# microsoft/fadtk

Hardware: AMD Instinct MI355X
Metric: FAD scores/sec + cov-GEMM TFLOP/s (% MFMA peak), N=100k D=512 (higher is better)
Workload: dtype f16 in, f16 MFMA with f32 accumulate over <= 8192-row runs, f64 across runs (moments); split-f16 MFMA iterations (f32 accumulate) + exact int8-MFMA products (int32 accumulate) + f64 correction (Frechet)

## Files before the change

### fadtk_amd/csrc/moments_kernels.h

```cpp
#pragma once
#include "fad_common.h"
#include <type_traits>

namespace fad {

typedef float f32x16 __attribute__((ext_vector_type(16)));
typedef double f64x4 __attribute__((ext_vector_type(4)));
typedef _Float16 f16x8 __attribute__((ext_vector_type(8)));
typedef __bf16 bf16x8 __attribute__((ext_vector_type(8)));
typedef short s16x4 __attribute__((ext_vector_type(4)));

constexpr int kXcd = 8;
constexpr int kMaxSets = 16;
constexpr int kMaxSets256 = 32;

__device__ __forceinline__ int xcd_contiguous(int b, int nwg) {
    const int xcd = b % kXcd, idx = b / kXcd;
    const int q = nwg / kXcd, r = nwg % kXcd;
    return (xcd < r ? xcd * (q + 1) : r * (q + 1) + (xcd - r) * q) + idx;
}

__device__ __forceinline__ void tile_coords(int tile, int nt, int& ta, int& tb) {
    int a = 0, t = tile;
    while (t >= nt - a) { t -= nt - a; ++a; }
    ta = a; tb = a + t;
}

struct SegRun;
struct TileSet {
    const void* E;
    int64_t n, ld;
    int64_t rows_per_split;
    int S;
    int item0;
    void* partials;
    double* colpart;
    int* flag;
    uint16_t* cvec;
    const SegRun* runs;
    const int* split_first_run;
    float* seg_runsum;
};
struct SegRun { int64_t r0; int32_t rows; int32_t seg; };
struct TileLaunch {
    TileSet set[kMaxSets];
    int nsets, d, nt, T, total;
};

__device__ __forceinline__ const TileSet& locate(const TileLaunch& L, int w, int& split, int& tile, int64_t& k_begin,
                                                 int64_t& k_end, int& run_lo, int& run_hi) {
    int si = 0;
#pragma unroll
    for (int i = 1; i < kMaxSets; ++i)
        if (i < L.nsets && w >= L.set[i].item0) si = i;
    const TileSet& s = L.set[si];
    const int local = w - s.item0;
    split = local / L.T; tile = local - split * L.T;
    k_begin = (int64_t)split * s.rows_per_split;
    k_end = (k_begin + s.rows_per_split < s.n) ? k_begin + s.rows_per_split : s.n;
    run_lo = 0; run_hi = 0;
    if (s.runs) { run_lo = s.split_first_run[split]; run_hi = s.split_first_run[split + 1]; }
    return s;
}

template <int KIND> __device__ __forceinline__ float h16_to_f32(uint32_t bits16) {
    if constexpr (KIND == FAD_F16) {
        _Float16 h; unsigned short s = (unsigned short)bits16; __builtin_memcpy(&h, &s, 2); return (float)h;
    } else {
        return __uint_as_float(bits16 << 16);
    }
}

template <int KIND> __device__ __forceinline__ float sum8(const uint4& v) {
    float s = 0.f;
    const uint32_t w[4] = {v.x, v.y, v.z, v.w};
#pragma unroll
    for (int q = 0; q < 4; ++q) {
        if constexpr (KIND == FAD_F16) {
            typedef _Float16 h2 __attribute__((ext_vector_type(2)));
            h2 a; __builtin_memcpy(&a, &w[q], 4);
            const h2 one = {(_Float16)1.0f, (_Float16)1.0f};
            s = __builtin_amdgcn_fdot2(a, one, s, false);
        } else {
            typedef __bf16 b2 __attribute__((ext_vector_type(2)));
            b2 a, one; __builtin_memcpy(&a, &w[q], 4);
            const uint32_t ob = 0x3f803f80u; __builtin_memcpy(&one, &ob, 4);
            s = __builtin_amdgcn_fdot2_f32_bf16(a, one, s, false);
        }
    }
    return s;
}

template <int KIND> __device__ __forceinline__ f32x16 mfma_h16(const uint4& a, const uint4& b, const f32x16& c) {
    if constexpr (KIND == FAD_F16) {
        f16x8 va, vb; __builtin_memcpy(&va, &a, 16); __builtin_memcpy(&vb, &b, 16);
        return __builtin_amdgcn_mfma_f32_32x32x16_f16(va, vb, c, 0, 0, 0);
    } else {
        bf16x8 va, vb; __builtin_memcpy(&va, &a, 16); __builtin_memcpy(&vb, &b, 16);
        return __builtin_amdgcn_mfma_f32_32x32x16_bf16(va, vb, c, 0, 0, 0);
    }
}

constexpr int H_BT = 128;
constexpr int H_TS = H_BT * H_BT + 64;
constexpr int H_KB = 32;
constexpr int H_NST = 4;

__device__ __attribute__((aligned(16))) uint4 g_zero16 = {0u, 0u, 0u, 0u};

typedef const void __attribute__((address_space(1)))* gptr_t;
typedef void __attribute__((address_space(3)))* lptr_t;

template <int N> __device__ __forceinline__ void wait_vmcnt() {
    asm volatile("s_waitcnt vmcnt(%0)" ::"n"(N) : "memory");
}

template <int N> __device__ __forceinline__ void wait_vmcnt_upto(int outstanding_steps) {
    switch (outstanding_steps) {
        case 0: wait_vmcnt<0>(); break;
        case 1: wait_vmcnt<N>(); break;
        case 2: wait_vmcnt<2 * N>(); break;
        case 3: wait_vmcnt<3 * N>(); break;
        case 4: wait_vmcnt<4 * N>(); break;
        case 5: wait_vmcnt<5 * N>(); break;
        case 6: wait_vmcnt<6 * N>(); break;
        default: wait_vmcnt<7 * N>(); break;
    }
}

template <int KIND, int NST, bool DIAG, bool FAST, bool SHIFT = false, bool WALK = false>
__device__ __forceinline__ void tile_h16_tr_body(
    const uint16_t* __restrict__ E, int64_t k_begin0, int64_t k_end0, int64_t ld, int d, int nt, int T,
    int split, int tile, int ca, int cb, float* __restrict__ partials, double* __restrict__ colpart,
    uint4* smem, int* __restrict__ shift_flag, const SegRun* __restrict__ runs, int run_lo, int run_hi,
    uint16_t* __restrict__ cvec = nullptr, float* __restrict__ seg_runsum = nullptr) {
    static_assert(!WALK || (DIAG && !SHIFT), "the per-file walk rides on the diagonal tiles of the first pass");
    static_assert(!SHIFT || KIND == FAD_F16, "the shifted pass is written for float16 rows");
    constexpr int LPS = DIAG ? 2 : 4;
    constexpr int STAGE = FAST ? 2 * H_KB * 16 : H_KB * 16;
    static_assert(FAST || DIAG, "single-tile launches only have the diagonal tile");
    const int tid = threadIdx.x, lane = tid & 63;
    const int wave = __builtin_amdgcn_readfirstlane(tid >> 6);
    const int wr = wave >> 1, wc = wave & 1;
    const int li = lane & 31, kg = lane >> 5;
    int64_t k_begin = k_begin0, k_end = k_end0;
    int nkb = 0;

    const int sr = tid >> 4, sc = (tid & 15) ^ (((tid >> 4) & 3) << 2);
    const bool col_ok_a = (ca + sc * 8) < d;
    const bool col_ok_b = (cb + sc * 8) < d;
    const uint16_t* ga = E + ca + sc * 8;
    const uint16_t* gb = E + cb + sc * 8;
    const uint16_t* zsrc = reinterpret_cast<const uint16_t*>(&g_zero16);
    const int t16 = lane & 15, grp = lane >> 4;
    const int tr_row = 8 * (grp >> 1) + (t16 >> 2);
    const int tr_col = 16 * (grp & 1) + 4 * (t16 & 3);

    auto issue_part = [&](int kb, int g) {
        uint4* st = smem + (kb % NST) * STAGE;
        const int h = DIAG ? g : (g >> 1);
        const int64_t r = k_begin + (int64_t)kb * H_KB + sr + 16 * h;
        const bool ok = r < k_end;
        const bool side_b = !DIAG && (g & 1);
        const uint16_t* src = side_b ? ((ok && col_ok_b) ? gb + r * ld : zsrc) : ((ok && col_ok_a) ? ga + r * ld : zsrc);
        uint4* dstp = st + 256 * h + 64 * wave + (side_b ? H_KB * 16 : 0);
        if (FAST) {
            const uint32_t m0v = __builtin_amdgcn_readfirstlane((uint32_t)(size_t)(lptr_t)dstp);
            asm volatile("s_mov_b32 m0, %1\n\ts_nop 0\n\tglobal_load_lds_dwordx4 %0, off" ::"v"(src), "s"(m0v) : "memory", "m0");
        } else {
            __builtin_amdgcn_global_load_lds((gptr_t)src, (lptr_t)dstp, 16, 0, 0);
        }
    };
    auto issue = [&](int kb) {
#pragma unroll
        for (int g = 0; g < LPS; ++g) issue_part(kb, g);
    };
    const bool cols_full = (ca + H_BT <= d) && (cb + H_BT <= d) && ld < ((int64_t)1 << 26);
    const uint32_t voff = (uint32_t)(((int64_t)sr * ld + sc * 8) * 2);
    const uint32_t smem_lds = (uint32_t)(size_t)(lptr_t)smem;
    auto issue_fast = [&](int kb) {
#pragma unroll
        for (int g = 0; g < LPS; ++g) {
            const int h = DIAG ? g : (g >> 1);
            const bool side_b = !DIAG && (g & 1);
            const uint64_t sb = (uint64_t)(E + (k_begin + (int64_t)kb * H_KB + 16 * h) * ld + (side_b ? cb : ca));
            const uint32_t lo = __builtin_amdgcn_readfirstlane((uint32_t)sb);
            const uint32_t hi = __builtin_amdgcn_readfirstlane((uint32_t)(sb >> 32));
            const uint64_t ub = ((uint64_t)hi << 32) | lo;
            const uint32_t dst = smem_lds + (uint32_t)(((kb % NST) * STAGE + 256 * h + 64 * wave + (side_b ? H_KB * 16 : 0)) * 16);
            const uint32_t m0v = __builtin_amdgcn_readfirstlane(dst);
            asm volatile("s_mov_b32 m0, %2\n\ts_nop 0\n\tglobal_load_lds_dwordx4 %0, %1" ::"v"(voff), "s"(ub), "s"(m0v) : "memory", "m0");
        }
    };
    int nfast = 0;

    f32x16 acc[2][2];
#pragma unroll
    for (int x = 0; x < 2; ++x)
#pragma unroll
        for (int y = 0; y < 2; ++y)
#pragma unroll
            for (int q = 0; q < 16; ++q) acc[x][y][q] = 0.f;
    double csum[2] = {0.0, 0.0};
    double ctot[2] = {0.0, 0.0};
    const bool do_colsum = DIAG && (wr == wc);

    auto frag = [&](const char* slab, int ks, int col0) -> uint4 {
        const int r0 = ks * 16 + tr_row, r1 = r0 + 4, col = col0 + tr_col;
        const int o0 = r0 * 256 + (((col >> 3) ^ ((r0 & 3) << 2)) << 4) + ((col >> 2) & 1) * 8;
        const int o1 = r1 * 256 + (((col >> 3) ^ ((r1 & 3) << 2)) << 4) + ((col >> 2) & 1) * 8;
        const s16x4 lo = __builtin_amdgcn_ds_read_tr16_b64_v4i16((__attribute__((address_space(3))) s16x4*)(slab + o0));
        const s16x4 hi = __builtin_amdgcn_ds_read_tr16_b64_v4i16((__attribute__((address_space(3))) s16x4*)(slab + o1));
        uint4 f;
        __builtin_memcpy(&f.x, &lo, 8);
        __builtin_memcpy(&f.z, &hi, 8);
        return f;
    };
    auto split2 = [&](uint4 f, uint32_t c2, int64_t rows_left, uint4& xs, uint4& es) {
        typedef _Float16 h2 __attribute__((ext_vector_type(2)));
        uint32_t w[4] = {f.x, f.y, f.z, f.w}, x[4], e[4];
        h2 c; __builtin_memcpy(&c, &c2, 4);
        const h2 b = -c;
#pragma unroll
        for (int q = 0; q < 4; ++q) {
            h2 a; __builtin_memcpy(&a, &w[q], 4);
            const h2 sm = a + b;
            const h2 bb = sm - a;
            const h2 er = (a - (sm - bb)) + (b - bb);
            __builtin_memcpy(&x[q], &sm, 4);
            __builtin_memcpy(&e[q], &er, 4);
            if (rows_left < 8) {
                const uint32_t m = ((2 * q < rows_left) ? 0xffffu : 0u) | ((2 * q + 1 < rows_left) ? 0xffff0000u : 0u);
                x[q] &= m; e[q] &= m;
            }
        }
        xs = make_uint4(x[0], x[1], x[2], x[3]);
        es = make_uint4(e[0], e[1], e[2], e[3]);
    };
    uint32_t cs[4] = {0u, 0u, 0u, 0u};
    if constexpr (SHIFT) {
        const uint16_t* cv = cvec + (int64_t)split * (nt * H_BT);
        const bool four = DIAG && (wr != wc);
        const int col[4] = {four ? ca + li : ca + 64 * wr + li, four ? ca + 32 + li : ca + 64 * wr + 32 + li,
                            four ? ca + 64 + li : cb + 64 * wc + li, four ? ca + 96 + li : cb + 64 * wc + 32 + li};
#pragma unroll
        for (int q = 0; q < 4; ++q) { const uint32_t h = cv[col[q]]; cs[q] = h | (h << 16); }
    }
    auto rows_left_at = [&](int kb, int ks) -> int64_t { return k_end - (k_begin + (int64_t)kb * H_KB + ks * 16 + 8 * kg); };
    auto load_frags = [&](int kb, int ks, uint4 (&F)[4], uint4 (&R)[4], bool full) {
        const char* sA = reinterpret_cast<const char*>(smem + (kb % NST) * STAGE);
        const char* sB = DIAG ? sA : sA + H_KB * 256;
        F[0] = frag(sA, ks, 64 * wr); F[1] = frag(sA, ks, 64 * wr + 32);
// ... 1062 lines not shown
```

### fadtk_amd/csrc/moments_tile256.h

```cpp
#pragma once
#include "moments_kernels.h"
#include "tile256_roles.h"

namespace fad {

constexpr int T2_KB = 32;
#ifndef T2_NST_VALUE
#define T2_NST_VALUE 4
#endif
constexpr int T2_NST = T2_NST_VALUE;
constexpr int T2_ROW = 1024;
constexpr int T2_STAGE = T2_KB * T2_ROW;
constexpr size_t kT256Lds = (size_t)T2_NST * T2_STAGE;

struct T256Set {
    const void* E; int64_t n, ld, rows_per_split;
    int S, item0;
    float* partials;
    double* colpart;
    int* flag;
    uint16_t* cvec;
    const int32_t* idx; int64_t n_src;
};
struct T256Launch {
    T256Set set[kMaxSets256];
    int nsets, d, nsb, NT, total;
    uint8_t type[t256::MAX_TYPES], sa[t256::MAX_TYPES], sb[t256::MAX_TYPES];
};

__device__ __forceinline__ void t2_phase_barrier() {
    __builtin_amdgcn_sched_barrier(0);
    __builtin_amdgcn_s_barrier();
    __builtin_amdgcn_sched_barrier(0);
}

__device__ __forceinline__ uint4 t2_frag(uint32_t lds_byte) {
    typedef __attribute__((address_space(3))) s16x4* lp_t;
    const s16x4 lo = __builtin_amdgcn_ds_read_tr16_b64_v4i16((lp_t)(size_t)lds_byte);
    const s16x4 hi = __builtin_amdgcn_ds_read_tr16_b64_v4i16((lp_t)(size_t)(lds_byte + 4 * T2_ROW));
    uint4 f;
    __builtin_memcpy(&f.x, &lo, 8);
    __builtin_memcpy(&f.z, &hi, 8);
    return f;
}

__device__ __forceinline__ void t2_split2(const uint4& f, uint32_t c2, int64_t rows_left, uint4& xs, uint4& es) {
    typedef _Float16 h2 __attribute__((ext_vector_type(2)));
    uint32_t w[4] = {f.x, f.y, f.z, f.w}, x[4], e[4];
    h2 c; __builtin_memcpy(&c, &c2, 4);
    const h2 b = -c;
#pragma unroll
    for (int q = 0; q < 4; ++q) {
        h2 a; __builtin_memcpy(&a, &w[q], 4);
        const h2 sm = a + b;
        const h2 bb = sm - a;
        const h2 er = (a - (sm - bb)) + (b - bb);
        __builtin_memcpy(&x[q], &sm, 4);
        __builtin_memcpy(&e[q], &er, 4);
        if (rows_left < 8) {
            const uint32_t m = ((2 * q < rows_left) ? 0xffffu : 0u) | ((2 * q + 1 < rows_left) ? 0xffff0000u : 0u);
            x[q] &= m; e[q] &= m;
        }
    }
    xs = make_uint4(x[0], x[1], x[2], x[3]);
    es = make_uint4(e[0], e[1], e[2], e[3]);
}

template <int KIND, int ROLE, bool SHIFT, bool IDX>
__device__ __forceinline__ void tile256_wave(
    const T256Launch& L, const T256Set& s, int split, int ti, int type, int sa, int sb, const t256::WaveJob job, char* smem) {
    using RD = t256::RoleDef<ROLE>;
    constexpr int NF = RD::NF, NB = RD::NB;
    static_assert(!SHIFT || KIND == FAD_F16, "the shifted pass is written for float16 rows");
    constexpr int NSTG = T2_NST;
    constexpr int LPS = 4;
    const int tid = threadIdx.x, lane = tid & 63;
    const int wave = __builtin_amdgcn_readfirstlane(tid >> 6);
    const int quartet = wave >> 2;
    const int li = lane & 31, kg = lane >> 5;
    const uint16_t* __restrict__ E = static_cast<const uint16_t*>(s.E);
    const int64_t ld = s.ld;
    const int d = L.d;
    const bool two_rows = type == t256::TYPE_Z;
    const int64_t k_begin = (int64_t)split * s.rows_per_split;
    const int64_t k_end = (k_begin + s.rows_per_split < s.n) ? k_begin + s.rows_per_split : s.n;
    const int rows_per_stage = two_rows ? 2 * T2_KB : T2_KB;
    const int nkb = (int)((k_end - k_begin + rows_per_stage - 1) / rows_per_stage);
    const int colA = t256::SB * sa, colB = t256::SB * (two_rows ? sa : sb);
    const int my_rowoff = two_rows ? T2_KB * quartet : 0;

    typedef int srd_t __attribute__((ext_vector_type(4)));
    srd_t srd;
    {
        const uint64_t b = (uint64_t)(IDX ? E : E + k_begin * ld);
        const uint64_t nbytes = (uint64_t)(((IDX ? s.n_src : k_end - k_begin) - 1) * ld + d) * 2;
        srd[0] = __builtin_amdgcn_readfirstlane((int)(uint32_t)b);
        srd[1] = __builtin_amdgcn_readfirstlane((int)((uint32_t)(b >> 32) & 0xffffu));
        srd[2] = __builtin_amdgcn_readfirstlane((int)(uint32_t)nbytes);
        srd[3] = 0x00020000;
    }
    uint32_t voff[LPS];
    bool lane_in_b[LPS];
#pragma unroll
    for (int p = 0; p < LPS; ++p) {
        const int c = lane ^ (p << 2);
        const bool in_b = c >= 32;
        lane_in_b[p] = in_b;
        const int col = in_b ? colB + (c - 32) * 8 : colA + c * 8;
        const int64_t row = IDX ? 0 : LPS * wave + p + ((in_b && two_rows) ? T2_KB : 0);
        voff[p] = col < d ? (uint32_t)((row * ld + col) * 2) : 0x80000000u;
    }
    const uint32_t stage_bytes = (uint32_t)__builtin_amdgcn_readfirstlane((int)(uint32_t)((int64_t)rows_per_stage * ld * 2));
    const uint32_t row_bytes = (uint32_t)__builtin_amdgcn_readfirstlane((int)(uint32_t)(ld * 2));
    const uint32_t smem_lds = (uint32_t)(size_t)(lptr_t)smem;
    const uint32_t wave_lds = __builtin_amdgcn_readfirstlane(smem_lds + (uint32_t)(LPS * wave * T2_ROW));
    struct StageRows { uint32_t ro[LPS], ro2[LPS]; };
    auto rows_of_stage = [&](int kb) -> StageRows {
        StageRows r;
        if constexpr (IDX) {
            const int64_t p0 = k_begin + (int64_t)kb * rows_per_stage + LPS * wave;
#pragma unroll
            for (int p = 0; p < LPS; ++p) {
                const int64_t q = p0 + p, q2 = q + T2_KB;
                r.ro[p] = q < k_end ? (uint32_t)s.idx[q] * row_bytes : 0x80000000u;
                r.ro2[p] = (two_rows && q2 < k_end) ? (uint32_t)s.idx[q2 < k_end ? q2 : q] * row_bytes : 0x80000000u;
            }
        } else {
#pragma unroll
            for (int p = 0; p < LPS; ++p) { r.ro[p] = (uint32_t)kb * stage_bytes; r.ro2[p] = r.ro[p]; }
        }
        return r;
    };
    auto piece = [&](int kb, int p, const StageRows& r) {
#ifdef T2_ABL_NODMA
        if (kb >= NSTG - 1) return;
#endif
        uint32_t vo;
        if constexpr (IDX) vo = voff[p] + ((two_rows && lane_in_b[p]) ? r.ro2[p] : r.ro[p]);
        else vo = voff[p] + r.ro[p];
        const uint32_t m0v = wave_lds + (uint32_t)((kb % NSTG) * T2_STAGE + p * T2_ROW);
#ifdef T2_NT
        asm volatile("s_mov_b32 m0, %2\n\ts_nop 0\n\tbuffer_load_dwordx4 %0, %1, 0 offen nt lds" ::"v"(vo), "s"(srd), "s"(m0v) : "memory");
#else
        asm volatile("s_mov_b32 m0, %2\n\ts_nop 0\n\tbuffer_load_dwordx4 %0, %1, 0 offen lds" ::"v"(vo), "s"(srd), "s"(m0v) : "memory");
#endif
    };
    auto issue = [&](int kb) {
        const StageRows r = rows_of_stage(kb);
#pragma unroll
        for (int p = 0; p < LPS; ++p) piece(kb, p, r);
    };
    const int nwhole = (int)((k_end - k_begin) / rows_per_stage);

    const int t16 = lane & 15, grp = lane >> 4;
    const int tr_row = 8 * (grp >> 1) + (t16 >> 2), tr_col = 16 * (grp & 1) + 4 * (t16 & 3);
    auto frag_of = [&](int i, bool& from_a) -> int {
        if constexpr (ROLE == t256::XR) {
            from_a = i < 4;
            return from_a ? job.a0 + i : job.b0 + (i - 4);
        } else {
            from_a = job.slab == 0;
            return RD::frag[i];
        }
    };
    auto fcol = [&](int i) -> int {
        bool from_a; const int f = frag_of(i, from_a);
        return (from_a ? colA : colB) + 32 * f + li;
    };
    uint32_t foff[NF];
#pragma unroll
    for (int i = 0; i < NF; ++i) {
        bool from_a; const int f = frag_of(i, from_a);
        const int col = (from_a ? 0 : t256::SB) + 32 * f + tr_col;
        foff[i] = (uint32_t)(tr_row * T2_ROW + (((col >> 3) ^ ((tr_row & 3) << 2)) << 4) + ((col >> 2) & 1) * 8);
    }
    uint32_t cs[NF];
#pragma unroll
    for (int i = 0; i < NF; ++i) cs[i] = 0u;
    if constexpr (SHIFT) {
        const uint16_t* cv = s.cvec + (int64_t)split * (L.nsb * t256::SB);
#pragma unroll
        for (int i = 0; i < NF; ++i) { const uint32_t h = cv[fcol(i)]; cs[i] = h | (h << 16); }
    }
    auto rows_left_at = [&](int kb, int ks) -> int64_t {
        return k_end - (k_begin + (int64_t)kb * rows_per_stage + my_rowoff + ks * 16 + 8 * kg);
    };

    f32x16 acc[NB];
#pragma unroll
    for (int b = 0; b < NB; ++b)
#pragma unroll
        for (int q = 0; q < 16; ++q) acc[b][q] = 0.f;
    constexpr bool CSUM = ROLE != t256::XR;
    constexpr int CS0 = (ROLE == t256::TRI_HI || ROLE == t256::RECT_C) ? 2 : 0;
    double csum[2] = {0.0, 0.0};

    uint4 F0[NF], F1[NF];
    auto load_half = [&](int kb, int ks, uint4 (&F)[NF]) {
#ifdef T2_ABL_NOREAD
        if (kb > 0) return;
#endif
        const uint32_t base = smem_lds + (uint32_t)((kb % NSTG) * T2_STAGE + ks * 16 * T2_ROW);
#pragma unroll
        for (int i = 0; i < NF; ++i) F[i] = t2_frag(base + foff[i]);
    };
    auto half = [&](int kb, int ks, const uint4 (&F)[NF], auto refill, const StageRows& rr) {
        constexpr int PH = LPS / 2;
        if constexpr (SHIFT) {
            if (decltype(refill)::value) { piece(kb + NSTG - 1, PH * ks, rr); piece(kb + NSTG - 1, PH * ks + 1, rr); }
            const bool full = kb < nwhole;
            uint4 X[NF], R[NF];
#pragma unroll
            for (int i = 0; i < NF; ++i) t2_split2(F[i], cs[i], full ? 8 : rows_left_at(kb, ks), X[i], R[i]);
#pragma unroll
            for (int b = 0; b < NB; ++b) {
                acc[b] = mfma_h16<KIND>(X[RD::fa[b]], X[RD::fb[b]], acc[b]);
                acc[b] = mfma_h16<KIND>(X[RD::fa[b]], R[RD::fb[b]], acc[b]);
                acc[b] = mfma_h16<KIND>(R[RD::fa[b]], X[RD::fb[b]], acc[b]);
            }
            if constexpr (CSUM) {
#pragma unroll
                for (int i = 0; i < 2; ++i) csum[i] += (double)sum8<KIND>(X[CS0 + i]) + (double)sum8<KIND>(R[CS0 + i]);
            }
            return;
        }
#ifdef T2_ABL_NOMMA
#pragma unroll
        for (int i = 0; i < NF; ++i) acc[0][i] += __uint_as_float((F[i].x ^ F[i].y ^ F[i].z ^ F[i].w) & 0x007fffffu);
        if (decltype(refill)::value) { piece(kb + NSTG - 1, PH * ks, rr); piece(kb + NSTG - 1, PH * ks + 1, rr); }
        return;
#endif
#pragma unroll
        for (int b = 0; b < NB; ++b) {
            acc[b] = mfma_h16<KIND>(F[RD::fa[b]], F[RD::fb[b]], acc[b]);
            if (decltype(refill)::value && (b & 1) && (b >> 1) < PH) {
                __builtin_amdgcn_sched_barrier(0); piece(kb + NSTG - 1, PH * ks + (b >> 1), rr); __builtin_amdgcn_sched_barrier(0);
            }
#ifndef T2_OPT_NOCOLSUM
            if constexpr (CSUM) {
                if (b == 4 || b == 6) {
                    const int i = (b - 4) >> 1;
                    csum[i] += (double)sum8<KIND>(F[CS0 + i]);
                }
            }
#endif
        }
    };
    auto wait_next = [&](int kb) {
        const int last = (kb + NSTG - 1 < nkb - 1) ? kb + NSTG - 1 : nkb - 1;
        wait_vmcnt_upto<LPS>(last - (kb + 1));
    };
    static_assert(NSTG <= 8 && NSTG >= 3, "wait_vmcnt_upto counts at most seven stages");

    for (int s0 = 0; s0 < NSTG - 1 && s0 < nkb; ++s0) issue(s0);
    wait_vmcnt_upto<LPS>(((nkb < NSTG - 1) ? nkb : NSTG - 1) - 1);
    t2_phase_barrier();
    load_half(0, 0, F0);
    const int hot = nkb - (NSTG - 1) > 0 ? nkb - (NSTG - 1) : 0;
    int kb = 0;
    for (; kb < hot; ++kb) {
        const StageRows rr = rows_of_stage(kb + NSTG - 1);
        load_half(kb, 1, F1);
        __builtin_amdgcn_sched_barrier(0);
        half(kb, 0, F0, std::true_type{}, rr);
        __builtin_amdgcn_sched_barrier(0);
        asm volatile("s_waitcnt vmcnt(%0) lgkmcnt(0)" ::"n"(LPS * (NSTG - 3) + LPS / 2) : "memory");
        t2_phase_barrier();
        load_half(kb + 1, 0, F0);
        __builtin_amdgcn_sched_barrier(0);
        half(kb, 1, F1, std::true_type{}, rr);
        __builtin_amdgcn_sched_barrier(0);
    }
    const StageRows none = rows_of_stage(0);
    for (; kb < nkb; ++kb) {
        load_half(kb, 1, F1);
        __builtin_amdgcn_sched_barrier(0);
        half(kb, 0, F0, std::false_type{}, none);
        __builtin_amdgcn_sched_barrier(0);
        asm volatile("s_waitcnt lgkmcnt(0)" ::: "memory");
        const bool more = kb + 1 < nkb;
        if (more) {
            wait_next(kb);
            t2_phase_barrier();
            load_half(kb + 1, 0, F0);
            __builtin_amdgcn_sched_barrier(0);
        }
        half(kb, 1, F1, std::false_type{}, none);
        __builtin_amdgcn_sched_barrier(0);
    }

    {
        float4* out = reinterpret_cast<float4*>(s.partials + ((int64_t)split * L.NT + ti) * t256::ITEM_STRIDE) + (size_t)(9 * wave) * 256;
#pragma unroll
        for (int b = 0; b < NB; ++b)
#pragma unroll
            for (int q = 0; q < 4; ++q)
                out[(b * 4 + q) * 64 + lane] = make_float4(acc[b][4 * q], acc[b][4 * q + 1], acc[b][4 * q + 2], acc[b][4 * q + 3]);
    }

    float s2col[2] = {0.f, 0.f};
    if constexpr (!SHIFT) {
        if (s.flag) {
            float* dsq = reinterpret_cast<float*>(smem) + quartet * t256::SB;
            __syncthreads();
            if constexpr (CSUM) {
#pragma unroll
                for (int b = 0; b < NB; ++b) {
                    if (RD::fa[b] != RD::fb[b]) continue;
                    float v = 0.f;
#pragma unroll
                    for (int q = 0; q < 4; ++q)
#pragma unroll
                        for (int j = 0; j < 4; ++j)
                            if ((li >> 3) == q && (li & 3) == j) v = acc[b][4 * q + j];
                    if (kg == ((li >> 2) & 1)) dsq[32 * RD::frag[RD::fa[b]] + li] = v;
                }
            }
            __syncthreads();
            if constexpr (CSUM) {
#pragma unroll
                for (int i = 0; i < 2; ++i) s2col[i] = dsq[32 * RD::frag[CS0 + i] + li];
            }
        }
    }

    if constexpr (CSUM) {
        const int dpad = L.nsb * t256::SB;
        const int half_ = (two_rows && job.slab) ? 1 : 0;
        double* cp = s.colpart + ((int64_t)split * 2 + half_) * dpad;
        int64_t my_rows = k_end - k_begin;
        if (two_rows) {
            const int64_t whole = my_rows / 64, rem = my_rows - whole * 64;
            my_rows = whole * 32 + (half_ ? (rem > 32 ? rem - 32 : 0) : (rem < 32 ? rem : 32));
        }
        bool hit = false;
#pragma unroll
        for (int i = 0; i < 2; ++i) {
            const int col = fcol(CS0 + i);
            double sx = csum[i];
            sx += __shfl_xor(sx, 32);
            if (kg == 0) cp[col] = sx;
            if constexpr (!SHIFT) {
                if (s.flag) {
                    const double s2 = (double)s2col[i];
                    const double nr = (double)my_rows;
                    const double mean = sx / nr, var = s2 / nr - mean * mean;
                    const bool col_in = col < d;
                    hit = hit || (col_in && nr > 0.0 && !(mean * mean <= 64.0 * var) && !(sx == 0.0 && s2 == 0.0));
                    if (s.cvec && kg == 0 && half_ == 0) {
                        const bool worth = col_in && nr > 0.0 && (mean * mean > var) && (mean == mean) && !isinf(mean) && fabs(mean) < 65000.0;
                        const _Float16 ch = worth ? (_Float16)(float)mean : (_Float16)0.0f;
                        uint16_t bits; __builtin_memcpy(&bits, &ch, 2);
                        s.cvec[(int64_t)split * dpad + col] = bits;
                    }
                }
            }
        }
        if constexpr (!SHIFT) {
            if (s.flag && __any(hit) && lane == 0) atomicOr(s.flag, 1);
        }
    }
}

template <int KIND, bool SHIFT, bool IDX = false>
__global__ __launch_bounds__(512) __attribute__((amdgpu_num_vgpr(112))) void moments_tile256(T256Launch L) {
    extern __shared__ __attribute__((aligned(16))) uint4 smem_dyn[];
    char* const smem_bytes = reinterpret_cast<char*>(smem_dyn);
    const int w = xcd_contiguous(blockIdx.x, L.total);
    int si = 0;
#pragma unroll
    for (int i = 1; i < kMaxSets256; ++i)
        if (i < L.nsets && w >= L.set[i].item0) si = i;
    const T256Set& s = L.set[si];
    if constexpr (SHIFT) {
        if (!s.flag || *s.flag == 0) return;
    }
    const int local = w - s.item0;
    const int split = local / L.NT, ti = local - split * L.NT;
    const int type = L.type[ti], sa = L.sa[ti], sb = L.sb[ti];
    const int wave = __builtin_amdgcn_readfirstlane(threadIdx.x >> 6);
    const t256::WaveJob job = t256::wave_job(type, wave);
    switch (job.role) {
        case t256::TRI_LO: tile256_wave<KIND, t256::TRI_LO, SHIFT, IDX>(L, s, split, ti, type, sa, sb, job, smem_bytes); break;
        case t256::TRI_HI: tile256_wave<KIND, t256::TRI_HI, SHIFT, IDX>(L, s, split, ti, type, sa, sb, job, smem_bytes); break;
        case t256::RECT_C: tile256_wave<KIND, t256::RECT_C, SHIFT, IDX>(L, s, split, ti, type, sa, sb, job, smem_bytes); break;
        case t256::RECT_D: tile256_wave<KIND, t256::RECT_D, SHIFT, IDX>(L, s, split, ti, type, sa, sb, job, smem_bytes); break;
        default: tile256_wave<KIND, t256::XR, SHIFT, IDX>(L, s, split, ti, type, sa, sb, job, smem_bytes); break;
    }
}

struct R256Job {
    const float* partials; const double* colpart; const uint16_t* cvec;
    double* acc; double n_add;
    const int* gate; int* clear_flag;
    int S, overwrite;
    int64_t rows_per_split, n_rows;
};
struct R256Launch {
    R256Job job[kMaxSets256];
    const t256::BlockSrc* table;
    int d, nsb, NT, nblk, sl;
    uint32_t two_mask;
};

__global__ __launch_bounds__(256) void moments_reduce256(R256Launch R) {
    __shared__ double red[256 * 4];
    const R256Job& j = R.job[blockIdx.y];
    if (j.clear_flag && blockIdx.x == 0 && threadIdx.x == 0) *j.clear_flag = 0;
    const bool unshift = j.gate && *j.gate != 0 && j.cvec;
    const int SL = R.sl, G = 256 / SL;
    const int dpad = R.nsb * t256::SB;
    const int tile_blocks = (R.nblk * 256 + G - 1) / G;
    const int block = blockIdx.x;
    const int S = j.S;
    auto rows_of = [&](int sp) -> double {
        const int64_t left = j.n_rows - (int64_t)sp * j.rows_per_split;
        return (double)(left < j.rows_per_split ? left : j.rows_per_split);
    };
    if (block >= tile_blocks) {
        const int a = (block - tile_blocks) * 64 + (threadIdx.x & 63), l = threadIdx.x >> 6;
        if (block == tile_blocks && threadIdx.x == 0) j.acc[0] = j.overwrite ? j.n_add : j.acc[0] + j.n_add;
        double t = 0.0;
        if (a < R.d) {
            const bool two = (R.two_mask >> (a / t256::SB)) & 1u;
            const double* cp = j.colpart + a;
            int sp = l;
            for (; sp + 28 < S; sp += 32) {
                double v[8], w[8];
#pragma unroll
                for (int u = 0; u < 8; ++u) { v[u] = cp[((int64_t)(sp + 4 * u) * 2) * dpad]; w[u] = two ? cp[((int64_t)(sp + 4 * u) * 2 + 1) * dpad] : 0.0; }
#pragma unroll
                for (int u = 0; u < 8; ++u) t += v[u] + w[u];
            }
            for (; sp < S; sp += 4) t += cp[((int64_t)sp * 2) * dpad] + (two ? cp[((int64_t)sp * 2 + 1) * dpad] : 0.0);
            if (unshift)
                for (int q = l; q < S; q += 4) t += rows_of(q) * f16_bits_to_f64(j.cvec[(int64_t)q * dpad + a]);
        }
        red[threadIdx.x] = t;
        __syncthreads();
        if (l == 0 && a < R.d) {
            const double tot = (red[threadIdx.x] + red[threadIdx.x + 64]) + (red[threadIdx.x + 128] + red[threadIdx.x + 192]);
            j.acc[1 + a] = j.overwrite ? tot : j.acc[1 + a] + tot;
        }
        return;
    }
    const int sl = threadIdx.x / G, gl = threadIdx.x % G;
    const int64_t g = (int64_t)block * G + gl;
    const bool live = g < (int64_t)R.nblk * 256;
    double s[4] = {0.0, 0.0, 0.0, 0.0};
    int bi = 0, bj = 0, e = 0;
    if (live) {
        const int ob = (int)(g >> 8);
        e = (int)(g & 255);
        const int nb = t256::NFR * R.nsb;
        int rem = ob;
        while (rem >= nb - bi) { rem -= nb - bi; ++bi; }
        bj = bi + rem;
        const t256::BlockSrc src = R.table[ob];
        const int64_t stride = (int64_t)R.NT * t256::ITEM_STRIDE;
#pragma unroll
        for (int h = 0; h < 2; ++h) {
            if (src.src[h] < 0) continue;
            const int ti = src.src[h] / t256::SLOTS, slot = src.src[h] - ti * t256::SLOTS;
            const float* p = j.partials + (int64_t)ti * t256::ITEM_STRIDE + (int64_t)slot * t256::BLK + e * 4;
            int sp = sl;
#ifdef R256_ABL_NOLOAD
            sp = S;
#endif
            for (; sp + 7 * SL < S; sp += 8 * SL) {
                float4 v[8];
#pragma unroll
                for (int u = 0; u < 8; ++u) v[u] = *reinterpret_cast<const float4*>(p + (sp + u * SL) * stride);
#pragma unroll
                for (int u = 0; u < 8; u += 2) {
                    s[0] += (double)v[u].x + (double)v[u + 1].x; s[1] += (double)v[u].y + (double)v[u + 1].y;
                    s[2] += (double)v[u].z + (double)v[u + 1].z; s[3] += (double)v[u].w + (double)v[u + 1].w;
                }
            }
            for (; sp < S; sp += SL) {
                const float4 v = *reinterpret_cast<const float4*>(p + sp * stride);
                s[0] += (double)v.x; s[1] += (double)v.y; s[2] += (double)v.z; s[3] += (double)v.w;
            }
        }
        if (unshift) {
            const int ga = 32 * bi + 8 * (e >> 6) + 4 * ((e & 63) >> 5), gb = 32 * bj + (e & 31);
            const bool two_a = (R.two_mask >> (ga / t256::SB)) & 1u, two_b = (R.two_mask >> (gb / t256::SB)) & 1u;
            for (int sp = sl; sp < S; sp += SL) {
                const double nq = rows_of(sp);
                const uint16_t* cv = j.cvec + (int64_t)sp * dpad;
                const double* sv = j.colpart + ((int64_t)sp * 2) * dpad;
                const double cb_ = f16_bits_to_f64(cv[gb]), sb_ = sv[gb] + (two_b ? sv[dpad + gb] : 0.0);
#pragma unroll
                for (int q = 0; q < 4; ++q) {
                    const double ca_ = f16_bits_to_f64(cv[ga + q]), sa_ = sv[ga + q] + (two_a ? sv[dpad + ga + q] : 0.0);
                    s[q] += ca_ * sb_ + sa_ * cb_ + nq * ca_ * cb_;
                }
            }
        }
    }
    if (SL > 1) {
#pragma unroll
        for (int q = 0; q < 4; ++q) red[(sl * G + gl) * 4 + q] = s[q];
        __syncthreads();
        if (sl != 0) return;
#pragma unroll
        for (int q = 0; q < 4; ++q) {
            double t = 0.0;
            for (int l = 0; l < SL; ++l) t += red[(l * G + gl) * 4 + q];
            s[q] = t;
        }
    }
    if (!live) return;
#ifdef R256_ABL_NOWRITE
    if (s[0] + s[1] + s[2] + s[3] == 12345.678) j.acc[1] = 0.0;
    return;
#endif
    double* M = j.acc + 1 + R.d;
    const int d = R.d;
    const int a0 = 32 * bi + 8 * (e >> 6) + 4 * ((e & 63) >> 5), b = 32 * bj + (e & 31);
    if (b >= d) return;
#pragma unroll
    for (int q = 0; q < 4; ++q) {
        const int a = a0 + q;
        if (a >= d) continue;
        const int64_t ab = (int64_t)a * d + b, ba = (int64_t)b * d + a;
        if (bi != bj) {
            M[ab] = j.overwrite ? s[q] : M[ab] + s[q];
            M[ba] = j.overwrite ? s[q] : M[ba] + s[q];
        } else if (a <= b) {
            M[ab] = j.overwrite ? s[q] : M[ab] + s[q];
            if (a != b) M[ba] = j.overwrite ? s[q] : M[ba] + s[q];
        }
    }
}

}
```

Measured before the change: 12360.

## Switch tile256 GEMM to 16x16x32 MFMA sub-blocks with new LDS swizzle

Replaces each 32x32x16 MFMA accumulator with four 16x16x32 sub-block accumulators and reorganizes the stage processing into first/mid/last quarters. The LDS swizzle, DMA chunk mapping, fragment offsets and output slot layout move into a new layout header. On diagonal blocks the redundant lower sub-block MFMA is skipped. The aim is to use the MFMA shape with higher throughput per instruction, cut diagonal work and reduce LDS bank conflicts. The cost is more accumulator registers, reworked column-sum and diagonal extraction, and a changed schedule for refill placement.

Result: faster. 12900 (median of 6 runs) (+4.4%).

```diff
diff --git a/fadtk_amd/csrc/moments_kernels.h b/fadtk_amd/csrc/moments_kernels.h
--- a/fadtk_amd/csrc/moments_kernels.h
+++ b/fadtk_amd/csrc/moments_kernels.h
@@ -5,6 +5,7 @@
 namespace fad {
 
 typedef float f32x16 __attribute__((ext_vector_type(16)));
+typedef float f32x4 __attribute__((ext_vector_type(4)));
 typedef double f64x4 __attribute__((ext_vector_type(4)));
 typedef _Float16 f16x8 __attribute__((ext_vector_type(8)));
 typedef __bf16 bf16x8 __attribute__((ext_vector_type(8)));
@@ -98,6 +99,16 @@
     } else {
         bf16x8 va, vb; __builtin_memcpy(&va, &a, 16); __builtin_memcpy(&vb, &b, 16);
         return __builtin_amdgcn_mfma_f32_32x32x16_bf16(va, vb, c, 0, 0, 0);
+    }
+}
+
+template <int KIND> __device__ __forceinline__ f32x4 mfma16_h16(const uint4& a, const uint4& b, const f32x4& c) {
+    if constexpr (KIND == FAD_F16) {
+        f16x8 va, vb; __builtin_memcpy(&va, &a, 16); __builtin_memcpy(&vb, &b, 16);
+        return __builtin_amdgcn_mfma_f32_16x16x32_f16(va, vb, c, 0, 0, 0);
+    } else {
+        bf16x8 va, vb; __builtin_memcpy(&va, &a, 16); __builtin_memcpy(&vb, &b, 16);
+        return __builtin_amdgcn_mfma_f32_16x16x32_bf16(va, vb, c, 0, 0, 0);
     }
 }
 
diff --git a/fadtk_amd/csrc/moments_tile256.h b/fadtk_amd/csrc/moments_tile256.h
--- a/fadtk_amd/csrc/moments_tile256.h
+++ b/fadtk_amd/csrc/moments_tile256.h
@@ -1,6 +1,7 @@
 #pragma once
 #include "moments_kernels.h"
 #include "tile256_roles.h"
+#include "tile256_layout.h"
 
 namespace fad {
 
@@ -11,6 +12,7 @@
 constexpr int T2_NST = T2_NST_VALUE;
 constexpr int T2_ROW = 1024;
 constexpr int T2_STAGE = T2_KB * T2_ROW;
+static_assert(T2_KB == t256::STAGE_ROWS && T2_ROW == t256::ROW_BYTES, "tile256_layout.h describes this stage");
 constexpr size_t kT256Lds = (size_t)T2_NST * T2_STAGE;
 
 struct T256Set {
@@ -103,7 +105,7 @@
     bool lane_in_b[LPS];
 #pragma unroll
     for (int p = 0; p < LPS; ++p) {
-        const int c = lane ^ (p << 2);
+        const int c = t256::dma_chunk(wave, p, lane);
         const bool in_b = c >= 32;
         lane_in_b[p] = in_b;
         const int col = in_b ? colB + (c - 32) * 8 : colA + c * 8;
@@ -136,8 +138,10 @@
         if (kb >= NSTG - 1) return;
 #endif
         uint32_t vo;
-        if constexpr (IDX) vo = voff[p] + ((two_rows && lane_in_b[p]) ? r.ro2[p] : r.ro[p]);
-        else vo = voff[p] + r.ro[p];
+        if constexpr (IDX) {
+            const uint32_t ro = (two_rows && lane_in_b[p]) ? r.ro2[p] : r.ro[p];
+            vo = ((voff[p] | ro) & 0x80000000u) ? 0x80000000u : voff[p] + ro;
+        } else vo = voff[p] + r.ro[p];
         const uint32_t m0v = wave_lds + (uint32_t)((kb % NSTG) * T2_STAGE + p * T2_ROW);
 #ifdef T2_NT
         asm volatile("s_mov_b32 m0, %2\n\ts_nop 0\n\tbuffer_load_dwordx4 %0, %1, 0 offen nt lds" ::"v"(vo), "s"(srd), "s"(m0v) : "memory");
@@ -153,7 +157,6 @@
     const int nwhole = (int)((k_end - k_begin) / rows_per_stage);
 
     const int t16 = lane & 15, grp = lane >> 4;
-    const int tr_row = 8 * (grp >> 1) + (t16 >> 2), tr_col = 16 * (grp & 1) + 4 * (t16 & 3);
     auto frag_of = [&](int i, bool& from_a) -> int {
         if constexpr (ROLE == t256::XR) {
             from_a = i < 4;
@@ -163,87 +166,142 @@
             return RD::frag[i];
         }
     };
-    auto fcol = [&](int i) -> int {
+    auto fcol = [&](int i, int c32) -> int {
         bool from_a; const int f = frag_of(i, from_a);
-        return (from_a ? colA : colB) + 32 * f + li;
+        return (from_a ? colA : colB) + 32 * f + c32;
     };
     uint32_t foff[NF];
+    static_assert((t256::tr_read_byte(5, 0, 16) ^ t256::tr_read_byte(5, 0, 0)) == 32 && (t256::tr_read_byte(62, 1, 48) ^ t256::tr_read_byte(62, 1, 32)) == 32,
+                  "sub-fragment 1 = sub-fragment 0 ^ 32 bytes");
 #pragma unroll
     for (int i = 0; i < NF; ++i) {
         bool from_a; const int f = frag_of(i, from_a);
-        const int col = (from_a ? 0 : t256::SB) + 32 * f + tr_col;
-        foff[i] = (uint32_t)(tr_row * T2_ROW + (((col >> 3) ^ ((tr_row & 3) << 2)) << 4) + ((col >> 2) & 1) * 8);
-    }
-    uint32_t cs[NF];
-#pragma unroll
-    for (int i = 0; i < NF; ++i) cs[i] = 0u;
+        foff[i] = (uint32_t)t256::tr_read_byte(lane, 0, (from_a ? 0 : t256::SB) + 32 * f);
+    }
+    uint32_t cs[NF][2];
+#pragma unroll
+    for (int i = 0; i < NF; ++i) cs[i][0] = cs[i][1] = 0u;
     if constexpr (SHIFT) {
         const uint16_t* cv = s.cvec + (int64_t)split * (L.nsb * t256::SB);
 #pragma unroll
-        for (int i = 0; i < NF; ++i) { const uint32_t h = cv[fcol(i)]; cs[i] = h | (h << 16); }
-    }
-    auto rows_left_at = [&](int kb, int ks) -> int64_t {
-        return k_end - (k_begin + (int64_t)kb * rows_per_stage + my_rowoff + ks * 16 + 8 * kg);
-    };
-
-    f32x16 acc[NB];
+        for (int i = 0; i < NF; ++i)
+#pragma unroll
+            for (int sf = 0; sf < 2; ++sf) { const uint32_t h = cv[fcol(i, 16 * sf + t16)]; cs[i][sf] = h | (h << 16); }
+    }
+    auto rows_left_at = [&](int kb) -> int64_t {
+        return k_end - (k_begin + (int64_t)kb * rows_per_stage + my_rowoff + t256::lane_row0(lane));
+    };
+
+    f32x4 acc[NB][4];
 #pragma unroll
     for (int b = 0; b < NB; ++b)
 #pragma unroll
-        for (int q = 0; q < 16; ++q) acc[b][q] = 0.f;
+        for (int q = 0; q < 4; ++q) acc[b][q] = f32x4{0.f, 0.f, 0.f, 0.f};
     constexpr bool CSUM = ROLE != t256::XR;
     constexpr int CS0 = (ROLE == t256::TRI_HI || ROLE == t256::RECT_C) ? 2 : 0;
-    double csum[2] = {0.0, 0.0};
+    double csum[2][2] = {{0.0, 0.0}, {0.0, 0.0}};
 
     uint4 F0[NF], F1[NF];
-    auto load_half = [&](int kb, int ks, uint4 (&F)[NF]) {
+    auto load_sub = [&](int kb, int sf, uint4 (&F)[NF]) {
 #ifdef T2_ABL_NOREAD
         if (kb > 0) return;
 #endif
-        const uint32_t base = smem_lds + (uint32_t)((kb % NSTG) * T2_STAGE + ks * 16 * T2_ROW);
-#pragma unroll
-        for (int i = 0; i < NF; ++i) F[i] = t2_frag(base + foff[i]);
-    };
-    auto half = [&](int kb, int ks, const uint4 (&F)[NF], auto refill, const StageRows& rr) {
-        constexpr int PH = LPS / 2;
+        const uint32_t base = smem_lds + (uint32_t)((kb % NSTG) * T2_STAGE);
+#pragma unroll
+        for (int i = 0; i < NF; ++i) F[i] = t2_frag(base + (foff[i] ^ (uint32_t)(sf << 5)));
+    };
+    auto refill_piece = [&](auto refill, int kb, int p, const StageRows& rr) {
+        if constexpr (decltype(refill)::value) {
+            __builtin_amdgcn_sched_barrier(0); piece(kb + NSTG - 1, p, rr); __builtin_amdgcn_sched_barrier(0);
+        }
+    };
+    constexpr int P_FIRST = SHIFT ? 2 : 1;
+    constexpr bool EARLY_READS = !SHIFT;
+    uint4 X0[NF], R0[NF], X1[NF], R1[NF];
+    auto mma3 = [&](f32x4& c, const uint4& xa, const uint4& ra, const uint4& xb, const uint4& rb) {
+        c = mfma16_h16<KIND>(xa, xb, c);
+        c = mfma16_h16<KIND>(xa, rb, c);
+        c = mfma16_h16<KIND>(ra, xb, c);
+    };
+    auto split_sub = [&](int kb, int sf, const uint4 (&F)[NF], uint4 (&X)[NF], uint4 (&R)[NF]) {
+        const int64_t left = kb < nwhole ? 8 : rows_left_at(kb);
+#pragma unroll
+        for (int i = 0; i < NF; ++i) t2_split2(F[i], cs[i][sf], left, X[i], R[i]);
+    };
+    auto quarter_first = [&](int kb, auto refill, const StageRows& rr) {
         if constexpr (SHIFT) {
-            if (decltype(refill)::value) { piece(kb + NSTG - 1, PH * ks, rr); piece(kb + NSTG - 1, PH * ks + 1, rr); }
-            const bool full = kb < nwhole;
-            uint4 X[NF], R[NF];
-#pragma unroll
-            for (int i = 0; i < NF; ++i) t2_split2(F[i], cs[i], full ? 8 : rows_left_at(kb, ks), X[i], R[i]);
+            refill_piece(refill, kb, 0, rr); refill_piece(refill, kb, 1, rr);
+            split_sub(kb, 0, F0, X0, R0);
+#pragma unroll
+            for (int b = 0; b < NB; ++b) mma3(acc[b][0], X0[RD::fa[b]], R0[RD::fa[b]], X0[RD::fb[b]], R0[RD::fb[b]]);
+            return;
+        }
+#ifdef T2_ABL_NOMMA
+#pragma unroll
+        for (int i = 0; i < NF; ++i) acc[0][0][i & 3] += __uint_as_float((F0[i].x ^ F0[i].y ^ F0[i].z ^ F0[i].w) & 0x007fffffu);
+        refill_piece(refill, kb, 0, rr);
+        return;
+#endif
+#pragma unroll
+        for (int b = 0; b < NB; ++b) {
+            acc[b][0] = mfma16_h16<KIND>(F0[RD::fa[b]], F0[RD::fb[b]], acc[b][0]);
+            if (b == 3) refill_piece(refill, kb, 0, rr);
+        }
+    };
+    auto quarter_mid = [&](int kb, auto refill, const StageRows& rr) {
+        if constexpr (SHIFT) {
+            refill_piece(refill, kb, 2, rr); refill_piece(refill, kb, 3, rr);
+            split_sub(kb, 1, F1, X1, R1);
 #pragma unroll
             for (int b = 0; b < NB; ++b) {
-                acc[b] = mfma_h16<KIND>(X[RD::fa[b]], X[RD::fb[b]], acc[b]);
-                acc[b] = mfma_h16<KIND>(X[RD::fa[b]], R[RD::fb[b]], acc[b]);
-                acc[b] = mfma_h16<KIND>(R[RD::fa[b]], X[RD::fb[b]], acc[b]);
+                mma3(acc[b][1], X0[RD::fa[b]], R0[RD::fa[b]], X1[RD::fb[b]], R1[RD::fb[b]]);
+                if (t256::sub_block_issued(RD::fa[b] == RD::fb[b], 1, 0)) mma3(acc[b][2], X1[RD::fa[b]], R1[RD::fa[b]], X0[RD::fb[b]], R0[RD::fb[b]]);
             }
             if constexpr (CSUM) {
 #pragma unroll
-                for (int i = 0; i < 2; ++i) csum[i] += (double)sum8<KIND>(X[CS0 + i]) + (double)sum8<KIND>(R[CS0 + i]);
+                for (int i = 0; i < 2; ++i) {
+                    csum[i][0] += (double)sum8<KIND>(X0[CS0 + i]) + (double)sum8<KIND>(R0[CS0 + i]);
+                    csum[i][1] += (double)sum8<KIND>(X1[CS0 + i]) + (double)sum8<KIND>(R1[CS0 + i]);
+                }
             }
             return;
         }
 #ifdef T2_ABL_NOMMA
 #pragma unroll
-        for (int i = 0; i < NF; ++i) acc[0][i] += __uint_as_float((F[i].x ^ F[i].y ^ F[i].z ^ F[i].w) & 0x007fffffu);
-        if (decltype(refill)::value) { piece(kb + NSTG - 1, PH * ks, rr); piece(kb + NSTG - 1, PH * ks + 1, rr); }
+        for (int i = 0; i < NF; ++i) acc[0][1][i & 3] += __uint_as_float((F1[i].x ^ F1[i].y ^ F1[i].z ^ F1[i].w) & 0x007fffffu);
+        refill_piece(refill, kb, 1, rr); refill_piece(refill, kb, 2, rr);
         return;
 #endif
 #pragma unroll
         for (int b = 0; b < NB; ++b) {
-            acc[b] = mfma_h16<KIND>(F[RD::fa[b]], F[RD::fb[b]], acc[b]);
-            if (decltype(refill)::value && (b & 1) && (b >> 1) < PH) {
-                __builtin_amdgcn_sched_barrier(0); piece(kb + NSTG - 1, PH * ks + (b >> 1), rr); __builtin_amdgcn_sched_barrier(0);
-            }
+            acc[b][1] = mfma16_h16<KIND>(F0[RD::fa[b]], F1[RD::fb[b]], acc[b][1]);
+            if (t256::sub_block_issued(RD::fa[b] == RD::fb[b], 1, 0)) acc[b][2] = mfma16_h16<KIND>(F1[RD::fa[b]], F0[RD::fb[b]], acc[b][2]);
+            if (b == 1) refill_piece(refill, kb, 1, rr);
+            if (b == 5) refill_piece(refill, kb, 2, rr);
 #ifndef T2_OPT_NOCOLSUM
             if constexpr (CSUM) {
-                if (b == 4 || b == 6) {
-                    const int i = (b - 4) >> 1;
-                    csum[i] += (double)sum8<KIND>(F[CS0 + i]);
-                }
-            }
-#endif
+                if (b == 2) csum[0][0] += (double)sum8<KIND>(F0[CS0]);
+                if (b == 3) csum[0][1] += (double)sum8<KIND>(F1[CS0]);
+                if (b == 6) csum[1][0] += (double)sum8<KIND>(F0[CS0 + 1]);
+                if (b == 7) csum[1][1] += (double)sum8<KIND>(F1[CS0 + 1]);
+            }
+#endif
+        }
+    };
+    auto quarter_last = [&](int kb, auto refill, const StageRows& rr) {
+        if constexpr (SHIFT) {
+#pragma unroll
+            for (int b = 0; b < NB; ++b) mma3(acc[b][3], X1[RD::fa[b]], R1[RD::fa[b]], X1[RD::fb[b]], R1[RD::fb[b]]);
+            return;
+        }
+#ifdef T2_ABL_NOMMA
+        refill_piece(refill, kb, 3, rr);
+        return;
+#endif
+#pragma unroll
+        for (int b = 0; b < NB; ++b) {
+            acc[b][3] = mfma16_h16<KIND>(F1[RD::fa[b]], F1[RD::fb[b]], acc[b][3]);
+            if (b == 3) refill_piece(refill, kb, 3, rr);
         }
     };
     auto wait_next = [&](int kb) {
@@ -255,38 +313,51 @@
     for (int s0 = 0; s0 < NSTG - 1 && s0 < nkb; ++s0) issue(s0);
     wait_vmcnt_upto<LPS>(((nkb < NSTG - 1) ? nkb : NSTG - 1) - 1);
     t2_phase_barrier();
-    load_half(0, 0, F0);
+    load_sub(0, 0, F0);
     const int hot = nkb - (NSTG - 1) > 0 ? nkb - (NSTG - 1) : 0;
     int kb = 0;
     for (; kb < hot; ++kb) {
         const StageRows rr = rows_of_stage(kb + NSTG - 1);
-        load_half(kb, 1, F1);
-        __builtin_amdgcn_sched_barrier(0);
-        half(kb, 0, F0, std::true_type{}, rr);
-        __builtin_amdgcn_sched_barrier(0);
-        asm volatile("s_waitcnt vmcnt(%0) lgkmcnt(0)" ::"n"(LPS * (NSTG - 3) + LPS / 2) : "memory");
+        if constexpr (!EARLY_READS) __builtin_amdgcn_sched_barrier(0); else load_sub(kb, 1, F1);
+        __builtin_amdgcn_sched_barrier(0);
+        quarter_first(kb, std::true_type{}, rr);
+        __builtin_amdgcn_sched_barrier(0);
+        if constexpr (!EARLY_READS) load_sub(kb, 1, F1);
+        asm volatile("s_waitcnt vmcnt(%0) lgkmcnt(0)" ::"n"(LPS * (NSTG - 3) + P_FIRST) : "memory");
         t2_phase_barrier();
-        load_half(kb + 1, 0, F0);
-        __builtin_amdgcn_sched_barrier(0);
-        half(kb, 1, F1, std::true_type{}, rr);
-        __builtin_amdgcn_sched_barrier(0);
+        quarter_mid(kb, std::true_type{}, rr);
+        __builtin_amdgcn_sched_barrier(0);
+        if constexpr (EARLY_READS) load_sub(kb + 1, 0, F0);
+        __builtin_amdgcn_sched_barrier(0);
+        quarter_last(kb, std::true_type{}, rr);
+        __builtin_amdgcn_sched_barrier(0);
+        if constexpr (!EARLY_READS) { load_sub(kb + 1, 0, F0); __builtin_amdgcn_sched_barrier(0); }
     }
     const StageRows none = rows_of_stage(0);
     for (; kb < nkb; ++kb) {
-        load_half(kb, 1, F1);
-        __builtin_amdgcn_sched_barrier(0);
-        half(kb, 0, F0, std::false_type{}, none);
-        __builtin_amdgcn_sched_barrier(0);
+        if constexpr (EARLY_READS) load_sub(kb, 1, F1);
+        __builtin_amdgcn_sched_barrier(0);
+        quarter_first(kb, std::false_type{}, none);
+        __builtin_amdgcn_sched_barrier(0);
+        if constexpr (!EARLY_READS) load_sub(kb, 1, F1);
         asm volatile("s_waitcnt lgkmcnt(0)" ::: "memory");
         const bool more = kb + 1 < nkb;
         if (more) {
             wait_next(kb);
             t2_phase_barrier();
-            load_half(kb + 1, 0, F0);
+        }
+        quarter_mid(kb, std::false_type{}, none);
+        __builtin_amdgcn_sched_barrier(0);
+        if (EARLY_READS && more) {
+            load_sub(kb + 1, 0, F0);
             __builtin_amdgcn_sched_barrier(0);
         }
-        half(kb, 1, F1, std::false_type{}, none);
-        __builtin_amdgcn_sched_barrier(0);
+        quarter_last(kb, std::false_type{}, none);
+        __builtin_amdgcn_sched_barrier(0);
+        if (!EARLY_READS && more) {
+            load_sub(kb + 1, 0, F0);
+            __builtin_amdgcn_sched_barrier(0);
+        }
     }
 
     {
@@ -295,7 +366,7 @@
         for (int b = 0; b < NB; ++b)
 #pragma unroll
             for (int q = 0; q < 4; ++q)
-                out[(b * 4 + q) * 64 + lane] = make_float4(acc[b][4 * q], acc[b][4 * q + 1], acc[b][4 * q + 2], acc[b][4 * q + 3]);
+                out[b * 256 + t256::slot_float4(q >> 1, q & 1, lane)] = make_float4(acc[b][q][0], acc[b][q][1], acc[b][q][2], acc[b][q][3]);
     }
 
     float s2col[2] = {0.f, 0.f};
@@ -307,13 +378,14 @@
 #pragma unroll
                 for (int b = 0; b < NB; ++b) {
                     if (RD::fa[b] != RD::fb[b]) continue;
-                    float v = 0.f;
-#pragma unroll
-                    for (int q = 0; q < 4; ++q)
+                    if (t256::diag_lane(t16) == lane) {
+                        float v0 = 0.f, v1 = 0.f;
 #pragma unroll
                         for (int j = 0; j < 4; ++j)
-                            if ((li >> 3) == q && (li & 3) == j) v = acc[b][4 * q + j];
-                    if (kg == ((li >> 2) & 1)) dsq[32 * RD::frag[RD::fa[b]] + li] = v;
+                            if (t256::diag_comp(t16) == j) { v0 = acc[b][0][j]; v1 = acc[b][3][j]; }
+                        dsq[32 * RD::frag[RD::fa[b]] + t16] = v0;
+                        dsq[32 * RD::frag[RD::fa[b]] + 16 + t16] = v1;
+                    }
                 }
             }
             __syncthreads();
@@ -336,8 +408,9 @@
         bool hit = false;
 #pragma unroll
         for (int i = 0; i < 2; ++i) {
-            const int col = fcol(CS0 + i);
-            double sx = csum[i];
+            const int col = fcol(CS0 + i, li);
+            const bool hi16 = (lane & 16) != 0;
+            double sx = (hi16 ? csum[i][1] : csum[i][0]) + __shfl_xor(hi16 ? csum[i][0] : csum[i][1], 16);
             sx += __shfl_xor(sx, 32);
             if (kg == 0) cp[col] = sx;
             if constexpr (!SHIFT) {
@@ -483,7 +556,7 @@
             }
         }
         if (unshift) {
-            const int ga = 32 * bi + 8 * (e >> 6) + 4 * ((e & 63) >> 5), gb = 32 * bj + (e & 31);
+            const int ga = 32 * bi + t256::slot_row0(e), gb = 32 * bj + t256::slot_col(e);
             const bool two_a = (R.two_mask >> (ga / t256::SB)) & 1u, two_b = (R.two_mask >> (gb / t256::SB)) & 1u;
             for (int sp = sl; sp < S; sp += SL) {
                 const double nq = rows_of(sp);
@@ -517,7 +590,7 @@
 #endif
     double* M = j.acc + 1 + R.d;
     const int d = R.d;
-    const int a0 = 32 * bi + 8 * (e >> 6) + 4 * ((e & 63) >> 5), b = 32 * bj + (e & 31);
+    const int a0 = 32 * bi + t256::slot_row0(e), b = 32 * bj + t256::slot_col(e);
     if (b >= d) return;
 #pragma unroll
     for (int q = 0; q < 4; ++q) {
diff --git a/fadtk_amd/csrc/tile256_layout.h b/fadtk_amd/csrc/tile256_layout.h
--- /dev/null
+++ b/fadtk_amd/csrc/tile256_layout.h
@@ -0,0 +1,28 @@
+#pragma once
+#include <cstdint>
+
+namespace fad {
+namespace t256 {
+
+constexpr int STAGE_ROWS = 32;
+constexpr int ROW_BYTES = 1024;
+
+constexpr int swizzle_of_row(int row) { return ((row & 3) << 1) | (((row >> 3) & 1) << 3); }
+constexpr int swizzled_chunk(int row, int chunk) { return chunk ^ swizzle_of_row(row); }
+constexpr int stage_byte(int row, int col) { return row * ROW_BYTES + (swizzled_chunk(row, col >> 3) << 4) + (col & 7) * 2; }
+constexpr int dma_chunk(int wave, int piece, int lane) { return lane ^ swizzle_of_row(4 * wave + piece); }
+constexpr int lane_row0(int lane) { return 8 * (lane >> 4); }
+constexpr int tr_read_byte(int lane, int j, int col0) {
+    return stage_byte(lane_row0(lane) + 4 * j + ((lane & 15) >> 2), col0 + 4 * (lane & 3));
+}
+
+constexpr int slot_float4(int si, int sj, int lane) { return 64 * (2 * si + sj) + lane; }
+constexpr int slot_row0(int e) { return 16 * (e >> 7) + 4 * ((e & 63) >> 4); }
+constexpr int slot_col(int e) { return 16 * ((e >> 6) & 1) + (e & 15); }
+constexpr bool sub_block_issued(bool diagonal, int si, int sj) { return !(diagonal && si == 1 && sj == 0); }
+constexpr int diag_sub(int c) { return c >> 4; }
+constexpr int diag_lane(int c) { return 16 * ((c & 15) >> 2) + (c & 15); }
+constexpr int diag_comp(int c) { return c & 3; }
+
+}
+}
```
